# NoahVl/Explaining-In-Style-Reproducibility-Study

Hardware: AMD Instinct MI355X
Metric: StylEx G+D+enc train-step images/sec @256px (higher is better)
Workload: dtype bf16; 1 GPU; FFHQ-shaped 256x256 StylEx, batch 32/GPU, GAE=2 (noise+encoder micro-steps), GP every 4th step, ResNet-18 classifier; image_size=256, batch_per_gpu=32, start_step=0, gradient_accumulate_every=2, global_batch=32, parallelism=dp1

## Files before the change

### explaining-in-style-reproducibility-study_amd/csrc/conv_pipe.hip

```cpp
#include <hip/hip_runtime.h>
#include <stdint.h>
#include <stdlib.h>

#include "conv_prims.h"
#include "stylex_internal.h"

#ifndef PIPE_STORE_AUX
#define PIPE_STORE_AUX 0
#endif

struct StylexPipeArgs {
    int total_tiles;
    unsigned m_ntiles, m_tpi, m_tx;
    int dbg;
};

#ifdef STYLEX_PIPE_ABLATION
#define PIPE_DBG (pa.dbg)
#else
#define PIPE_DBG 0
#endif


namespace {

typedef StylexPipeArgs PipeArgs;

template <int NT>
struct PipeCfg {
    static constexpr int TH = NT == 128 ? 16 : 32;
    static constexpr int TW = 32, HWD = TW + 2, NP = (TH + 2) * HWD;
    static constexpr int H_PIECES = (NP + 31) / 32;
    static constexpr int H_STRIDE = H_PIECES * 1024;
    static constexpr int W_PIECES = 9 * NT / 32;
    static constexpr int W_STRIDE = W_PIECES * 1024;
    static constexpr int HS = 3, WS = 2;
    static constexpr int W_BASE = HS * H_STRIDE;
    static constexpr int BIAS_BASE = W_BASE + WS * W_STRIDE;
    static constexpr int DUMP_BASE = BIAS_BASE + 2048;
    static constexpr int SMEM = DUMP_BASE + 1024;
    static constexpr int HP_MAX = (H_PIECES + 7) / 8;
    static constexpr int WP_MAX = (W_PIECES + 7) / 8;
    static constexpr int RG = TH / 4;
};

__device__ __forceinline__ void lds_wait(bf16x8 (&av)[4], bf16x8 (&bv)[2]) {
    asm volatile("s_waitcnt lgkmcnt(0)" : "+v"(av[0]), "+v"(av[1]), "+v"(av[2]), "+v"(av[3]), "+v"(bv[0]), "+v"(bv[1]));
}
template <int HWD, int TAP>
__device__ __forceinline__ void tap_addr(int (&addr)[4], int a_base, unsigned& swz) {
    constexpr int kh = TAP / 3, kw = TAP % 3;
    asm volatile("" : "+v"(swz));
#pragma unroll
    for (int i = 0; i < 4; ++i) addr[i] = a_base + ((i + kh) * HWD + kw) * 32 + (int)(((swz >> ((i + kh) * 3 + kw)) & 1u) << 4);
}
template <int NT, int TAP>
__device__ __forceinline__ void load_tap(bf16x8 (&av)[4], bf16x8 (&bv)[2], const int (&addr)[4], int b_addr) {
    lds_read16<(TAP * NT) * 32>(bv[0], b_addr);
    lds_read16<(TAP * NT + 32) * 32>(bv[1], b_addr);
#pragma unroll
    for (int i = 0; i < 4; ++i) lds_read16<0>(av[i], addr[i]);
}

__device__ __forceinline__ void mfma8(f32x16 (&acc)[4][2], const bf16x8 (&av)[4], const bf16x8 (&bv)[2]) {
#pragma unroll
    for (int i = 0; i < 4; ++i)
#pragma unroll
        for (int j = 0; j < 2; ++j) mfma1(acc[i][j], bv[j], av[i]);
}

template <int NT, int EPI>
__global__ __launch_bounds__(512, 2) void conv3x3_pipe_kernel(ConvKParams p, PipeArgs pa) {
    using Cfg = PipeCfg<NT>;
    constexpr int TH = Cfg::TH, HWD = Cfg::HWD, NP = Cfg::NP, H_PIECES = Cfg::H_PIECES, H_STRIDE = Cfg::H_STRIDE;
    constexpr int W_PIECES = Cfg::W_PIECES, W_STRIDE = Cfg::W_STRIDE, W_BASE = Cfg::W_BASE;
    constexpr int HP_MAX = Cfg::HP_MAX, WP_MAX = Cfg::WP_MAX, RG = Cfg::RG;
    static_assert(WP_MAX + HP_MAX <= 9, "one DMA piece per tap");
    extern __shared__ __attribute__((aligned(16))) char smem[];
    const int tid = threadIdx.x, lane = tid & 63;
    const int wave = __builtin_amdgcn_readfirstlane(tid >> 6);
    const int H = p.Ho, W = p.Wo, C = p.Ck, N = p.N;
    const int n_tiles = N / NT;
    const int tiles_x = (W + 31) >> 5, tiles_y = (H + TH - 1) / TH;
    const int tpi = tiles_x * tiles_y;

    int xs, xn, bslot, nslots;
    xcd_tile_span(pa.total_tiles, xs, xn, bslot, nslots);
    if (bslot >= xn) return;
    for (int i = (bslot & 3) * (PIPE_DBG >> 8); i > 0; --i) __builtin_amdgcn_s_sleep(16);
    const int my_tiles = xcd_my_tiles(xn, bslot, nslots);
    const int nchunks = C >> 4;
    const int total = my_tiles * nchunks;

    auto decode = [&](int k, int& b, int& y0, int& x0, int& n0) {
        const int t = xs + bslot + k * nslots;
        int pt = fastdiv(t, pa.m_ntiles);
        n0 = (t - pt * n_tiles) * NT;
        b = fastdiv(pt, pa.m_tpi);
        pt -= b * tpi;
        const int ty = fastdiv(pt, pa.m_tx);
        y0 = ty * TH;
        x0 = (pt - ty * tiles_x) * 32;
    };

    const unsigned bytes_x = (unsigned)((long)p.B * H * W * C * 2);
    const unsigned bytes_w = (unsigned)((long)N * 9 * C * 2);
    const __amdgpu_buffer_rsrc_t rx = __builtin_amdgcn_make_buffer_rsrc(const_cast<float*>(p.a), 0, (int)bytes_x, 0x00020000);
    const __amdgpu_buffer_rsrc_t rw = __builtin_amdgcn_make_buffer_rsrc(const_cast<void*>(p.w), 0, (int)bytes_w, 0x00020000);
    constexpr unsigned OOB = 0x80000000u;

    const int lr = lane >> 1, pslot = lane & 1;
    const int half = pslot ^ ((lr >> 3) & 1);
    int h_dst[HP_MAX], w_dst[WP_MAX];
#pragma unroll
    for (int it = 0; it < HP_MAX; ++it) h_dst[it] = wave + 8 * it < H_PIECES ? (wave + 8 * it) * 1024 : -1;
    unsigned voff_h[HP_MAX];
    auto halo_voff = [&](int b, int y0, int x0) {
#pragma unroll
        for (int it = 0; it < HP_MAX; ++it) {
            const int piece = wave + 8 * it;
            const int hp = piece * 32 + lr;
            const int hh = hp / HWD, ww = hp - hh * HWD;
            const int y = y0 - 1 + hh, x = x0 - 1 + ww;
            const bool ok = piece < H_PIECES && hp < NP && y >= 0 && y < H && x >= 0 && x < W;
            voff_h[it] = ok ? ((unsigned)((b * H + y) * W + x) * (unsigned)C + (unsigned)half * 8u) * 2u : OOB;
        }
    };
    unsigned voff_w[WP_MAX];
#pragma unroll
    for (int it = 0; it < WP_MAX; ++it) {
        const int piece = wave + 8 * it;
        const int r = piece * 32 + lr;
        const int tap = r / NT, n = r - tap * NT;
        const int gt = p.flip_taps ? 8 - tap : tap;
        voff_w[it] = piece < W_PIECES ? ((unsigned)(n * 9 + gt) * (unsigned)C + (unsigned)half * 8u) * 2u : OOB;
        w_dst[it] = piece < W_PIECES ? piece * 1024 : -1;
    }
#define issue_h1(IT, STAGE, SOFF, MORE)                                                                              \
    dma16(rx, smem, h_dst[IT] >= 0 ? (STAGE) * H_STRIDE + h_dst[IT] : Cfg::DUMP_BASE, (MORE) ? voff_h[IT] : OOB, SOFF)
#define issue_w1(IT, WBUF, SOFF, MORE)                                                                               \
    dma16(rw, smem, w_dst[IT] >= 0 ? W_BASE + (WBUF) * W_STRIDE + w_dst[IT] : Cfg::DUMP_BASE, (MORE) ? voff_w[IT] : OOB, SOFF)

    const int rg = wave % RG, nh = wave / RG;
    const int li = lane & 31, lk = lane >> 5;
    const int a_row = (4 * rg) * HWD + li;
    int a_base = a_row * 32;
    unsigned swz = 0;
#pragma unroll
    for (int r = 0; r < 6; ++r)
#pragma unroll
        for (int kw = 0; kw < 3; ++kw) {
            const int t = a_row + r * HWD + kw;
            swz |= (unsigned)(((t >> 3) ^ lk) & 1) << (r * 3 + kw);
        }
    const int b_cur0 = W_BASE + (nh * 64 + li) * 32 + ((((li >> 3) ^ lk) & 1) << 4), b_cur1 = b_cur0 + W_STRIDE;

    if (EPI == 0 && (p.flags & STYLEX_EPI_BIAS) && tid < N) reinterpret_cast<float*>(smem + Cfg::BIAS_BASE)[tid] = p.bias[tid];

    f32x16 acc[4][2];
    auto zero_acc = [&]() {
#pragma unroll
        for (int i = 0; i < 4; ++i)
#pragma unroll
            for (int j = 0; j < 2; ++j)
#pragma unroll
                for (int e = 0; e < 16; ++e) acc[i][j][e] = 0.f;
    };
    zero_acc();

    const bool act = EPI == 0 && (p.flags & (STYLEX_EPI_LRELU | STYLEX_EPI_RELU)) != 0;
    const float slope = (p.flags & STYLEX_EPI_RELU) ? 0.f : 0.2f;
    const float gslope = p.res_scale;
    const bool mask_out = EPI == 0 && p.mask != nullptr;
    auto gatem = [&](unsigned u, unsigned bits) -> unsigned {
        const float a0 = __uint_as_float(u << 16), c0 = __uint_as_float(u & 0xffff0000u);
        f32x2_t t = {(bits & 1u) ? a0 : gslope * a0, (bits & 2u) ? c0 : gslope * c0};
        bf16x2_t r = __builtin_convertvector(t, bf16x2_t);
        return *reinterpret_cast<unsigned*>(&r);
    };
    auto gate2 = [&](unsigned u, unsigned g) -> unsigned {
        const float a0 = __uint_as_float(u << 16), c0 = __uint_as_float(u & 0xffff0000u);
        const float ga = __uint_as_float(g << 16), gc = __uint_as_float(g & 0xffff0000u);
        f32x2_t t = {ga > 0.f ? a0 : gslope * a0, gc > 0.f ? c0 : gslope * c0};
        bf16x2_t r = __builtin_convertvector(t, bf16x2_t);
        return *reinterpret_cast<unsigned*>(&r);
    };
    const unsigned bytes_y = (unsigned)((long)p.B * H * W * N * 2);
    const __amdgpu_buffer_rsrc_t ry = __builtin_amdgcn_make_buffer_rsrc(p.y, 0, (int)bytes_y, 0x00020000);
    const __amdgpu_buffer_rsrc_t rgate = __builtin_amdgcn_make_buffer_rsrc(const_cast<float*>(p.residual), 0, (int)bytes_y, 0x00020000);
    const __amdgpu_buffer_rsrc_t rmask = __builtin_amdgcn_make_buffer_rsrc(
        EPI == 2 ? const_cast<unsigned char*>(p.gate_mask) : p.mask, 0, (int)(bytes_y >> 4), 0x00020000);
    const unsigned rowb = (unsigned)(W * N) * 2u;
    auto pack2 = [](float a, float c) -> unsigned {
        f32x2_t t = {a, c};
        bf16x2_t r = __builtin_convertvector(t, bf16x2_t);
        return *reinterpret_cast<unsigned*>(&r);
    };
    const unsigned lane_off = (unsigned)(((4 * rg) * W + (lane & 7)) * N + nh * 64) * 2u +
                              (unsigned)(4 * ((lane >> 4) & 1) + 2 * ((lane >> 3) & 1) + (lane >> 5)) * 16u;
    const unsigned pixb8 = (unsigned)N * 16u;
    auto epilogue = [&](int b, int y0, int x0, int n0) {
        const int lh = lk;
        const int nb = n0 + nh * 64;
        const unsigned t_off = __builtin_amdgcn_readfirstlane((unsigned)((((long)(b * H + y0) * W + x0) * N + n0) * 2));
        const unsigned g_off = x0 + li < W ? (unsigned)(((4 * rg) * W + li) * N + nh * 64 + 8 * lh) * 2u : OOB;
#pragma unroll
        for (int i = 0; i < 4; ++i) {
            const bool row_ok = y0 + 4 * rg + i < H;
            const unsigned soff = t_off + i * rowb;
            u32x4 R[4];
#pragma unroll
            for (int j = 0; j < 2; ++j) {
                u32x4 gv[2];
                unsigned gm[2];
                if (EPI != 0) {
                    const unsigned voff = row_ok ? g_off : OOB;
#pragma unroll
                    for (int q = 0; q < 2; ++q) {
                        if (EPI == 1) gv[q] = __builtin_amdgcn_raw_buffer_load_b128(rgate, voff + (j * 64 + q * 32), soff, 0);
                        if (EPI == 2) gm[q] = __builtin_amdgcn_raw_buffer_load_b8(rmask, (voff >> 4) + (j * 4 + q * 2), soff >> 4, 0);
                    }
                }
                float4 b4[4];
#pragma unroll
                for (int g = 0; g < 4; ++g)
                    b4[g] = (EPI == 0 && (p.flags & STYLEX_EPI_BIAS))
                                ? *reinterpret_cast<const float4*>(smem + Cfg::BIAS_BASE + (nb + j * 32 + 8 * g + 4 * lh) * 4)
                                : make_float4(0.f, 0.f, 0.f, 0.f);
                unsigned P[4][2];
#pragma unroll
                for (int g = 0; g < 4; ++g) {
                    float v0 = acc[i][j][4 * g + 0] + b4[g].x, v1 = acc[i][j][4 * g + 1] + b4[g].y;
                    float v2 = acc[i][j][4 * g + 2] + b4[g].z, v3 = acc[i][j][4 * g + 3] + b4[g].w;
                    if (act) {
                        v0 = v0 > 0.f ? v0 : slope * v0;
                        v1 = v1 > 0.f ? v1 : slope * v1;
                        v2 = v2 > 0.f ? v2 : slope * v2;
                        v3 = v3 > 0.f ? v3 : slope * v3;
                    }
                    P[g][0] = pack2(v0, v1);
                    P[g][1] = pack2(v2, v3);
                }
#pragma unroll
                for (int g = 0; g < 4; g += 2)
#pragma unroll
                    for (int h = 0; h < 2; ++h) {
                        auto r = __builtin_amdgcn_permlane32_swap(P[g][h], P[g + 1][h], false, false);
                        P[g][h] = r[0];
                        P[g + 1][h] = r[1];
                    }
#pragma unroll
                for (int q = 0; q < 2; ++q) {
                    uint4 v = make_uint4(P[2 * q][0], P[2 * q][1], P[2 * q + 1][0], P[2 * q + 1][1]);
                    if (EPI == 1) {
                        v.x = gate2(v.x, gv[q].x);
                        v.y = gate2(v.y, gv[q].y);
                        v.z = gate2(v.z, gv[q].z);
                        v.w = gate2(v.w, gv[q].w);
                    } else if (EPI == 2) {
                        const unsigned m = gm[q];
                        v.x = gatem(v.x, m);
                        v.y = gatem(v.y, m >> 2);
                        v.z = gatem(v.z, m >> 4);
                        v.w = gatem(v.w, m >> 6);
                    }
                    if (mask_out && !(PIPE_DBG & 1))
                        __builtin_amdgcn_raw_buffer_store_b8((unsigned char)stylex_sign_bits8(v), rmask,
                                                             ((row_ok ? g_off : OOB) >> 4) + (j * 4 + q * 2), soff >> 4, 0);
                    R[2 * j + q] = u32x4{v.x, v.y, v.z, v.w};
                }
            }
#pragma unroll
            for (int j = 0; j < 2; ++j)
#pragma unroll
                for (int d = 0; d < 4; ++d) {
                    const unsigned a0 = R[2 * j][d], a1 = R[2 * j + 1][d];
                    R[2 * j][d] = (unsigned)__builtin_amdgcn_update_dpp((int)a0, (int)a1, 0x128, 0xF, 0xC, false);
                    R[2 * j + 1][d] = (unsigned)__builtin_amdgcn_update_dpp((int)a1, (int)a0, 0x128, 0xF, 0x3, false);
                }
#pragma unroll
            for (int q = 0; q < 2; ++q)
#pragma unroll
                for (int d = 0; d < 4; ++d) {
                    auto r = __builtin_amdgcn_permlane16_swap(R[q][d], R[2 + q][d], false, false);
                    R[q][d] = r[0];
                    R[2 + q][d] = r[1];
                }
            if (!(PIPE_DBG & 1)) {
#pragma unroll
                for (int k = 0; k < 4; ++k) {
                    const unsigned voff = (row_ok && x0 + 8 * k + (lane & 7) < W) ? lane_off : OOB;
                    __builtin_amdgcn_raw_buffer_store_b128(R[k], ry, voff, soff + k * pixb8, PIPE_STORE_AUX);
                    asm volatile("s_nop 1" : "+v"(R[k]) : : "memory");
                }
            }
        }
    };

    int hb, hy0, hx0, hn0;
    int h_k = 0, h_ch = 0, h_stage = 0;
    int w_k = 0, w_ch = 0, w_buf = 0, w_n0;
    int cb, cy0, cx0, cn0;
    decode(0, cb, cy0, cx0, cn0);
    hb = cb, hy0 = cy0, hx0 = cx0, hn0 = cn0;
    w_n0 = cn0;
    halo_voff(hb, hy0, hx0);
    auto adv_h = [&]() {
        h_stage = h_stage == 2 ? 0 : h_stage + 1;
        if (++h_ch == nchunks) {
            h_ch = 0;
            if (++h_k < my_tiles) {
                decode(h_k, hb, hy0, hx0, hn0);
                if (PIPE_DBG & 2) hb = 0, hy0 = 0, hx0 = 0;
                halo_voff(hb, hy0, hx0);
            }
        }
    };
    auto adv_w = [&]() {
        w_buf ^= 1;
        if (++w_ch == nchunks) {
            w_ch = 0;
            if (++w_k < my_tiles) {
                int b_, y_, x_;
                decode(w_k, b_, y_, x_, w_n0);
                if (PIPE_DBG & 4) w_n0 = 0;
            }
        }
    };
#pragma unroll
    for (int it = 0; it < HP_MAX; ++it) issue_h1(it, 0, 0u, true);
    adv_h();
#pragma unroll
    for (int it = 0; it < WP_MAX; ++it) issue_w1(it, 0, (unsigned)(w_n0 * 9 * C) * 2u, true);
    adv_w();
#pragma unroll
    for (int it = 0; it < HP_MAX; ++it) issue_h1(it, 1, (unsigned)h_ch * 32u, total > 1);
    if (total > 1) adv_h();

    int c_ch = 0, c_k = 0, c_stage = 0;
    bf16x8 avA[4], bvA[2], avB[4], bvB[2];
    int addr[4];
    tap_addr<HWD, 0>(addr, a_base, swz);
    wait_vmcnt<HP_MAX>();
    __builtin_amdgcn_s_barrier();
    asm volatile("" ::: "memory");
    load_tap<NT, 0>(avA, bvA, addr, b_cur0);
    tap_addr<HWD, 1>(addr, a_base, swz);
    auto next_stage = [&]() {
        a_base += c_stage == 2 ? -2 * H_STRIDE : H_STRIDE;
        c_stage = c_stage == 2 ? 0 : c_stage + 1;
    };
    constexpr int PPT = 2;
#define PIPE_DMA(TAP, MORE_W, MORE_H)                                                              \
    _Pragma("unroll") for (int q_ = (TAP) * PPT; q_ < (TAP) * PPT + PPT; ++q_) {                   \
        if (q_ < WP_MAX) issue_w1(q_, w_buf, w_soff, MORE_W);                                      \
        else if (q_ - WP_MAX < HP_MAX) issue_h1(q_ - WP_MAX, h_stage, h_soff, MORE_H);             \
    }
#define PIPE_TAP(TAP, AVC, BVC, AVN, BVN, BCUR, MORE_W, MORE_H) \
    lds_wait(AVC, BVC);                                        \
    load_tap<NT, TAP + 1>(AVN, BVN, addr, BCUR);               \
    __builtin_amdgcn_sched_barrier(0);                         \
    mfma8(acc, AVC, BVC);                                      \
    if (TAP == 7) next_stage();                                \
    tap_addr<HWD, (TAP + 2) % 9>(addr, a_base, swz);           \
    PIPE_DMA(TAP, MORE_W, MORE_H)                              \
    __builtin_amdgcn_sched_barrier(0);
#define PIPE_LAST(AVC, BVC, AVN, BVN, BNEXT)                   \
    lds_wait(AVC, BVC);                                        \
    if (PIPE_DBG & 8) wait_vmcnt<HP_MAX + 16>();                 \
    else wait_vmcnt<HP_MAX>();                                 \
    __builtin_amdgcn_s_barrier();                              \
    asm volatile("" ::: "memory");                             \
    load_tap<NT, 0>(AVN, BVN, addr, BNEXT);                    \
    __builtin_amdgcn_sched_barrier(0);                         \
    mfma8(acc, AVC, BVC);                                      \
    tap_addr<HWD, 1>(addr, a_base, swz);                       \
    __builtin_amdgcn_sched_barrier(0);
#define PIPE_CHUNK(A1, B1, A2, B2, BCUR, BNEXT, MORE_W, MORE_H)                                    \
    {                                                                                              \
        const bool mw_ = MORE_W, mh_ = MORE_H;                                                     \
        const unsigned w_soff = (unsigned)(w_n0 * 9 * C + w_ch * 16) * 2u, h_soff = (unsigned)h_ch * 32u; \
        PIPE_TAP(0, A1, B1, A2, B2, BCUR, mw_, mh_)                                                \
        PIPE_TAP(1, A2, B2, A1, B1, BCUR, mw_, mh_)                                                \
        PIPE_TAP(2, A1, B1, A2, B2, BCUR, mw_, mh_)                                                \
        PIPE_TAP(3, A2, B2, A1, B1, BCUR, mw_, mh_)                                                \
        PIPE_TAP(4, A1, B1, A2, B2, BCUR, mw_, mh_)                                                \
        PIPE_TAP(5, A2, B2, A1, B1, BCUR, mw_, mh_)                                                \
        PIPE_TAP(6, A1, B1, A2, B2, BCUR, mw_, mh_)                                                \
        PIPE_TAP(7, A2, B2, A1, B1, BCUR, mw_, mh_)                                                \
        PIPE_LAST(A1, B1, A2, B2, BNEXT)                                                           \
        if (mw_) adv_w();                                                                          \
        if (mh_) adv_h();                                                                          \
    }
    for (int g = 0; g < total; g += 2) {
        PIPE_CHUNK(avA, bvA, avB, bvB, b_cur0, b_cur1, g + 1 < total, g + 2 < total)
        PIPE_CHUNK(avB, bvB, avA, bvA, b_cur1, b_cur0, g + 2 < total, g + 3 < total)
        c_ch += 2;
        if (c_ch == nchunks) {
            c_ch = 0;
            asm volatile("s_nop 15\n\ts_nop 15"
                         : "+v"(acc[0][0]), "+v"(acc[0][1]), "+v"(acc[1][0]), "+v"(acc[1][1]), "+v"(acc[2][0]), "+v"(acc[2][1]),
                           "+v"(acc[3][0]), "+v"(acc[3][1]));
            epilogue(cb, cy0, cx0, cn0);
            if (++c_k < my_tiles) {
                decode(c_k, cb, cy0, cx0, cn0);
                zero_acc();
            }
        }
    }
#undef PIPE_CHUNK
#undef PIPE_LAST
#undef PIPE_TAP
#undef PIPE_DMA
#undef issue_h1
#undef issue_w1
    asm volatile("s_waitcnt lgkmcnt(0)" ::: "memory");
    wait_vmcnt<0>();
}

template <int NT, int EPI>
int launch_pipe(const ConvKParams& p, hipStream_t s) {
    using Cfg = PipeCfg<NT>;
    const hipError_t e = stylex_dynamic_lds_once<conv3x3_pipe_kernel<NT, EPI>>(Cfg::SMEM);
    if (e != hipSuccess) return (int)e;
    const int tiles_x = (p.Wo + 31) / 32, tiles_y = (p.Ho + Cfg::TH - 1) / Cfg::TH, n_tiles = p.N / NT;
    PipeArgs pa;
    pa.total_tiles = p.B * tiles_x * tiles_y * n_tiles;
    pa.m_ntiles = magic_of(n_tiles);
    pa.m_tpi = magic_of(tiles_x * tiles_y);
    pa.m_tx = magic_of(tiles_x);
#ifdef STYLEX_PIPE_ABLATION
    pa.dbg = getenv("STYLEX_PIPE_DBG") ? atoi(getenv("STYLEX_PIPE_DBG")) : 0;
#else
    pa.dbg = 0;
#endif
    stylex_note_kernel("conv3x3_pipe_kernel<%d, %d>", NT, EPI);
    hipLaunchKernelGGL((conv3x3_pipe_kernel<NT, EPI>), dim3((unsigned)stylex_cu_count()), dim3(512), Cfg::SMEM, s, p, pa);
    return (int)hipGetLastError();
}

template <int NT>
int launch_pipe_epi(const ConvKParams& p, hipStream_t s) {
    if (p.flags & STYLEX_EPI_GATE) return launch_pipe<NT, 1>(p, s);
    if (p.flags & STYLEX_EPI_GATE_MASK) return launch_pipe<NT, 2>(p, s);
    return launch_pipe<NT, 0>(p, s);
}

}

int stylex_launch_pipe(const ConvKParams& p, hipStream_t s) {
    const char* env = getenv("STYLEX_CONV_PIPE");
    if (env && env[0] == '0') return STYLEX_NOT_APPLICABLE;
    if (!p.act_bf16 || p.a_scale || p.s2d_c) return STYLEX_NOT_APPLICABLE;
    if (p.flags & ~(STYLEX_EPI_BIAS | STYLEX_EPI_LRELU | STYLEX_EPI_RELU | STYLEX_EPI_GATE | STYLEX_EPI_GATE_MASK | STYLEX_EPI_MASK_OUT))
        return STYLEX_NOT_APPLICABLE;
    if ((p.flags & STYLEX_EPI_GATE) && (!p.residual || (reinterpret_cast<uintptr_t>(p.residual) & 15))) return STYLEX_NOT_APPLICABLE;
    if (p.Ck < 64 || p.Ck % 32 != 0 || p.N % 64 != 0 || p.N > 512 || p.Wo < 32 || p.Ho < 16) return STYLEX_NOT_APPLICABLE;
    if ((reinterpret_cast<uintptr_t>(p.a) & 15) || (reinterpret_cast<uintptr_t>(p.w) & 15) || (reinterpret_cast<uintptr_t>(p.y) & 15))
        return STYLEX_NOT_APPLICABLE;
    if ((long)p.B * p.Ho * p.Wo * p.Ck * 2 >= (1l << 31) || (long)p.N * 9 * p.Ck * 2 >= (1l << 31) ||
        (long)p.B * p.Ho * p.Wo * p.N * 2 >= (1l << 31))
        return STYLEX_NOT_APPLICABLE;
    const bool n128 = p.N % 128 == 0 && !(env && env[0] == '6');
    if (!n128) {
        if (p.Ho < 32 && !(env && env[0] == '6')) return STYLEX_NOT_APPLICABLE;
        if (!(env && env[0] == '6') && ((p.flags & STYLEX_EPI_GATE) || (p.flip_taps && !p.flags && p.Ck == 64)))
            return STYLEX_NOT_APPLICABLE;
    }
    if (p.dry) return 0;
    if (n128) return launch_pipe_epi<128>(p, s);
    return launch_pipe_epi<64>(p, s);
}
```

### explaining-in-style-reproducibility-study_amd/csrc/conv_prims.h

```cpp
#pragma once
#include <hip/hip_runtime.h>

#include "act_io.h"

typedef float f32x16 __attribute__((ext_vector_type(16)));
typedef short bf16x8 __attribute__((ext_vector_type(8)));
typedef __bf16 bf16x2_t __attribute__((ext_vector_type(2)));
typedef float f32x2_t __attribute__((ext_vector_type(2)));
typedef unsigned u32x4 __attribute__((ext_vector_type(4)));
typedef __attribute__((address_space(3))) void* lds_void_ptr;

__device__ __forceinline__ void dma16(__amdgpu_buffer_rsrc_t r, char* smem, int lds_off, unsigned voff, unsigned soff = 0) {
    __builtin_amdgcn_raw_ptr_buffer_load_lds(r, (lds_void_ptr)(smem + lds_off), 16, voff, soff, 0, 0);
}

template <int N>
__device__ __forceinline__ void wait_vmcnt() {
    asm volatile("s_waitcnt vmcnt(%0)" ::"n"(N) : "memory");
}

template <int OFF>
__device__ __forceinline__ void lds_read16(bf16x8& dst, int addr) {
    asm volatile("ds_read_b128 %0, %1 offset:%2" : "=v"(dst) : "v"(addr), "n"(OFF));
}

__device__ __forceinline__ void mfma1(f32x16& acc, const bf16x8& a, const bf16x8& b) {
    asm volatile("v_mfma_f32_32x32x16_bf16 %0, %1, %2, %0" : "+v"(acc) : "v"(a), "v"(b));
}

__device__ __forceinline__ int fastdiv(int n, unsigned magic) { return magic ? (int)__umulhi((unsigned)n, magic) : n; }
inline unsigned magic_of(int d) { return d <= 1 ? 0u : (unsigned)(((1ull << 32) + (unsigned)d - 1) / (unsigned)d); }

__device__ __forceinline__ void xcd_tile_span(int total_tiles, int& xs, int& xn, int& bslot, int& nslots) {
    const int xcd = blockIdx.x & 7;
    bslot = blockIdx.x >> 3, nslots = gridDim.x >> 3;
    const int tq = total_tiles >> 3, tr = total_tiles & 7;
    xs = xcd * tq + (xcd < tr ? xcd : tr), xn = tq + (xcd < tr ? 1 : 0);
}
__device__ __forceinline__ int xcd_my_tiles(int xn, int bslot, int nslots) { return (xn - bslot + nslots - 1) / nslots; }
```

Measured before the change: 1003 images/sec.

## Add 16x16x32 MFMA variant of pipelined conv3x3 kernel for NT=128

New measurement: 1011 images/sec, median of 6. No clear change (+0.8%).

```diff
diff --git a/explaining-in-style-reproducibility-study_amd/csrc/conv_pipe.hip b/explaining-in-style-reproducibility-study_amd/csrc/conv_pipe.hip
--- a/explaining-in-style-reproducibility-study_amd/csrc/conv_pipe.hip
+++ b/explaining-in-style-reproducibility-study_amd/csrc/conv_pipe.hip
@@ -7,6 +7,10 @@
 
 #ifndef PIPE_STORE_AUX
 #define PIPE_STORE_AUX 0
+#endif
+
+#ifndef PIPE_MFMA
+#define PIPE_MFMA 0
 #endif
 
 struct StylexPipeArgs {
@@ -42,6 +46,7 @@
     static constexpr int HP_MAX = (H_PIECES + 7) / 8;
     static constexpr int WP_MAX = (W_PIECES + 7) / 8;
     static constexpr int RG = TH / 4;
+    static constexpr int mfma_n(int epi) { return PIPE_MFMA ? PIPE_MFMA : NT == 128 ? 16 : 32; }
 };
 
 __device__ __forceinline__ void lds_wait(bf16x8 (&av)[4], bf16x8 (&bv)[2]) {
@@ -70,7 +75,7 @@
 }
 
 template <int NT, int EPI>
-__global__ __launch_bounds__(512, 2) void conv3x3_pipe_kernel(ConvKParams p, PipeArgs pa) {
+__device__ __forceinline__ void pipe_body32(const ConvKParams& p, const PipeArgs& pa) {
     using Cfg = PipeCfg<NT>;
     constexpr int TH = Cfg::TH, HWD = Cfg::HWD, NP = Cfg::NP, H_PIECES = Cfg::H_PIECES, H_STRIDE = Cfg::H_STRIDE;
     constexpr int W_PIECES = Cfg::W_PIECES, W_STRIDE = Cfg::W_STRIDE, W_BASE = Cfg::W_BASE;
@@ -418,6 +423,424 @@
     wait_vmcnt<0>();
 }
 
+template <int HWD, int T>
+__device__ __forceinline__ void kstep_addr(int (&addr)[4], int a_base, int mid_delta, unsigned& swz, int& ls) {
+    constexpr int tA = (2 * T) % 9, tB = (2 * T + 1) % 9;
+    constexpr int offA = ((tA / 3) * HWD + tA % 3) * 32, offB = ((tB / 3) * HWD + tB % 3) * 32;
+    asm volatile("" : "+v"(swz), "+v"(ls));
+    const unsigned m = swz >> (tA + ls * (tB - tA));
+    int base = a_base + offA + ls * (offB - offA);
+    if (T == 4) base += ls * mid_delta;
+#pragma unroll
+    for (int i = 0; i < 4; ++i) addr[i] = base + i * HWD * 32 + (int)(((m >> (3 * i)) & 1u) << 4);
+}
+template <int OFF, int J0>
+__device__ __forceinline__ void load_w2(bf16x8 (&w)[4], int base) {
+    lds_read16<OFF + J0 * 512>(w[J0], base);
+    lds_read16<OFF + J0 * 512 + 512>(w[J0 + 1], base);
+}
+template <int I0>
+__device__ __forceinline__ void load_x4(bf16x8 (&x)[4], const int (&addr)[4]) {
+    lds_read16<0>(x[0], addr[I0]);
+    lds_read16<512>(x[1], addr[I0]);
+    lds_read16<0>(x[2], addr[I0 + 1]);
+    lds_read16<512>(x[3], addr[I0 + 1]);
+}
+__device__ __forceinline__ void lds_wait0(bf16x8 (&w)[4], bf16x8 (&x)[4]) {
+    asm volatile("s_waitcnt lgkmcnt(0)" : "+v"(w[0]), "+v"(w[1]), "+v"(w[2]), "+v"(w[3]), "+v"(x[0]), "+v"(x[1]), "+v"(x[2]), "+v"(x[3]));
+}
+__device__ __forceinline__ void lds_wait1(bf16x8 (&x)[4], bf16x8 (&wn)[4]) {
+    asm volatile("s_waitcnt lgkmcnt(0)" : "+v"(x[0]), "+v"(x[1]), "+v"(x[2]), "+v"(x[3]), "+v"(wn[0]), "+v"(wn[1]));
+}
+template <int P0>
+__device__ __forceinline__ void mfma16x16(f32x4 (&acc)[8][4], const bf16x8 (&w)[4], const bf16x8 (&x)[4]) {
+#pragma unroll
+    for (int q = 0; q < 4; ++q)
+#pragma unroll
+        for (int j = 0; j < 4; ++j) mfma16(acc[P0 + q][j], w[j], x[q]);
+}
+
+template <int NT, int EPI>
+__device__ __forceinline__ void pipe_body16(const ConvKParams& p, const PipeArgs& pa) {
+    using Cfg = PipeCfg<NT>;
+    constexpr int TH = Cfg::TH, HWD = Cfg::HWD, NP = Cfg::NP, H_PIECES = Cfg::H_PIECES, H_STRIDE = Cfg::H_STRIDE;
+    constexpr int W_PIECES = Cfg::W_PIECES, W_STRIDE = Cfg::W_STRIDE, W_BASE = Cfg::W_BASE;
+    constexpr int HP_MAX = Cfg::HP_MAX, WP_MAX = Cfg::WP_MAX, RG = Cfg::RG;
+    static_assert(WP_MAX + HP_MAX <= 9, "a phase's DMA pieces fit three half-steps");
+    extern __shared__ __attribute__((aligned(16))) char smem[];
+    const int tid = threadIdx.x, lane = tid & 63;
+    const int wave = __builtin_amdgcn_readfirstlane(tid >> 6);
+    const int H = p.Ho, W = p.Wo, C = p.Ck, N = p.N;
+    const int n_tiles = N / NT;
+    const int tiles_x = (W + 31) >> 5, tiles_y = (H + TH - 1) / TH;
+    const int tpi = tiles_x * tiles_y;
+
+    int xs, xn, bslot, nslots;
+    xcd_tile_span(pa.total_tiles, xs, xn, bslot, nslots);
+    if (bslot >= xn) return;
+    for (int i = (bslot & 3) * (PIPE_DBG >> 8); i > 0; --i) __builtin_amdgcn_s_sleep(16);
+    const int my_tiles = xcd_my_tiles(xn, bslot, nslots);
+    const int nchunks = C >> 4;
+    const int total = my_tiles * nchunks;
+
+    auto decode = [&](int k, int& b, int& y0, int& x0, int& n0) {
+        const int t = xs + bslot + k * nslots;
+        int pt = fastdiv(t, pa.m_ntiles);
+        n0 = (t - pt * n_tiles) * NT;
+        b = fastdiv(pt, pa.m_tpi);
+        pt -= b * tpi;
+        const int ty = fastdiv(pt, pa.m_tx);
+        y0 = ty * TH;
+        x0 = (pt - ty * tiles_x) * 32;
+    };
+
+    const unsigned bytes_x = (unsigned)((long)p.B * H * W * C * 2);
+    const unsigned bytes_w = (unsigned)((long)N * 9 * C * 2);
+    const __amdgpu_buffer_rsrc_t rx = __builtin_amdgcn_make_buffer_rsrc(const_cast<float*>(p.a), 0, (int)bytes_x, 0x00020000);
+    const __amdgpu_buffer_rsrc_t rw = __builtin_amdgcn_make_buffer_rsrc(const_cast<void*>(p.w), 0, (int)bytes_w, 0x00020000);
+    constexpr unsigned OOB = 0x80000000u;
+
+    const int lr = lane >> 1, pslot = lane & 1;
+    const int half = pslot ^ ((lr >> 3) & 1);
+    int h_dst[HP_MAX], w_dst[WP_MAX];
+#pragma unroll
+    for (int it = 0; it < HP_MAX; ++it) h_dst[it] = wave + 8 * it < H_PIECES ? (wave + 8 * it) * 1024 : -1;
+    unsigned voff_h[HP_MAX];
+    auto halo_voff = [&](int b, int y0, int x0) {
+#pragma unroll
+        for (int it = 0; it < HP_MAX; ++it) {
+            const int piece = wave + 8 * it;
+            const int hp = piece * 32 + lr;
+            const int hh = hp / HWD, ww = hp - hh * HWD;
+            const int y = y0 - 1 + hh, x = x0 - 1 + ww;
+            const bool ok = piece < H_PIECES && hp < NP && y >= 0 && y < H && x >= 0 && x < W;
+            voff_h[it] = ok ? ((unsigned)((b * H + y) * W + x) * (unsigned)C + (unsigned)half * 8u) * 2u : OOB;
+        }
+    };
+    unsigned voff_w[WP_MAX];
+#pragma unroll
+    for (int it = 0; it < WP_MAX; ++it) {
+        const int piece = wave + 8 * it;
+        const int r = piece * 32 + lr;
+        const int tap = r / NT, n = r - tap * NT;
+        const int gt = p.flip_taps ? 8 - tap : tap;
+        voff_w[it] = piece < W_PIECES ? ((unsigned)(n * 9 + gt) * (unsigned)C + (unsigned)half * 8u) * 2u : OOB;
+        w_dst[it] = piece < W_PIECES ? piece * 1024 : -1;
+    }
+#define issue_h1(IT, STAGE, SOFF, MORE)                                                                              \
+    dma16(rx, smem, h_dst[IT] >= 0 ? (STAGE) * H_STRIDE + h_dst[IT] : Cfg::DUMP_BASE, (MORE) ? voff_h[IT] : OOB, SOFF)
+#define issue_w1(IT, WBUF, SOFF, MORE)                                                                               \
+    dma16(rw, smem, w_dst[IT] >= 0 ? W_BASE + (WBUF) * W_STRIDE + w_dst[IT] : Cfg::DUMP_BASE, (MORE) ? voff_w[IT] : OOB, SOFF)
+
+    const int rg = wave % RG, nh = wave / RG;
+    const int lc = lane & 15, lh = (lane >> 4) & 1;
+    int ls = lane >> 5;
+    const int pc = lc ^ (lc < 8 ? 4 : 0);
+    const int a_row = (4 * rg) * HWD + pc;
+    int a_base = a_row * 32;
+    unsigned swz = 0;
+#pragma unroll
+    for (int r = 0; r < 6; ++r)
+#pragma unroll
+        for (int kw = 0; kw < 3; ++kw) {
+            const int t = a_row + r * HWD + kw;
+            swz |= (unsigned)(((t >> 3) ^ lh) & 1) << (r * 3 + kw);
+        }
+    const int b_0 = W_BASE + (nh * 64 + pc) * 32 + ((((pc >> 3) ^ lh) & 1) << 4);
+    const int b_s0 = b_0 + ls * (NT * 32), b_s1 = b_s0 + W_STRIDE;
+    const int b_mid = ls ? b_0 + W_STRIDE : b_0 + 8 * NT * 32;
+
+    if (EPI == 0 && (p.flags & STYLEX_EPI_BIAS) && tid < N) reinterpret_cast<float*>(smem + Cfg::BIAS_BASE)[tid] = p.bias[tid];
+
+    f32x4 acc[8][4];
+    auto zero_acc = [&]() {
+#pragma unroll
+        for (int q = 0; q < 8; ++q)
+#pragma unroll
+            for (int j = 0; j < 4; ++j)
+#pragma unroll
+                for (int e = 0; e < 4; ++e) acc[q][j][e] = 0.f;
+    };
+    zero_acc();
+
+    const bool act = EPI == 0 && (p.flags & (STYLEX_EPI_LRELU | STYLEX_EPI_RELU)) != 0;
+    const float slope = (p.flags & STYLEX_EPI_RELU) ? 0.f : 0.2f;
+    const float gslope = p.res_scale;
+    const bool mask_out = EPI == 0 && p.mask != nullptr;
+    auto gatem = [&](unsigned u, unsigned bits) -> unsigned {
+        const float a0 = __uint_as_float(u << 16), c0 = __uint_as_float(u & 0xffff0000u);
+        f32x2_t t = {(bits & 1u) ? a0 : gslope * a0, (bits & 2u) ? c0 : gslope * c0};
+        bf16x2_t r = __builtin_convertvector(t, bf16x2_t);
+        return *reinterpret_cast<unsigned*>(&r);
+    };
+    auto gate2 = [&](unsigned u, unsigned g) -> unsigned {
+        const float a0 = __uint_as_float(u << 16), c0 = __uint_as_float(u & 0xffff0000u);
+        const float ga = __uint_as_float(g << 16), gc = __uint_as_float(g & 0xffff0000u);
+        f32x2_t t = {ga > 0.f ? a0 : gslope * a0, gc > 0.f ? c0 : gslope * c0};
+        bf16x2_t r = __builtin_convertvector(t, bf16x2_t);
+        return *reinterpret_cast<unsigned*>(&r);
+    };
+    const unsigned bytes_y = (unsigned)((long)p.B * H * W * N * 2);
+    const __amdgpu_buffer_rsrc_t ry = __builtin_amdgcn_make_buffer_rsrc(p.y, 0, (int)bytes_y, 0x00020000);
+    const __amdgpu_buffer_rsrc_t rgate = __builtin_amdgcn_make_buffer_rsrc(const_cast<float*>(p.residual), 0, (int)bytes_y, 0x00020000);
+    const __amdgpu_buffer_rsrc_t rmask = __builtin_amdgcn_make_buffer_rsrc(
+        EPI == 2 ? const_cast<unsigned char*>(p.gate_mask) : p.mask, 0, (int)(bytes_y >> 4), 0x00020000);
+    const unsigned rowb = (unsigned)(W * N) * 2u;
+    auto pack2 = [](float a, float c) -> unsigned {
+        f32x2_t t = {a, c};
+        bf16x2_t r = __builtin_convertvector(t, bf16x2_t);
+        return *reinterpret_cast<unsigned*>(&r);
+    };
+    const bool lo32 = lane < 32;
+    const int quad = (lane >> 4) ^ (lane < 32 ? 1 : 0);
+    const unsigned g_base = (unsigned)(((4 * rg) * W + pc) * N + nh * 64) * 2u + (unsigned)(4 * lh + ls) * 16u;
+    const unsigned l_ch = (unsigned)(nh * 64) * 2u + (unsigned)(2 * ((lane >> 3) & 1) + 4 * lh + ls) * 16u;
+    const int px_t[2] = {(lane & 7) ^ 4, lane & 7};
+    const unsigned lane_off[2] = {(unsigned)(((4 * rg) * W + px_t[0]) * N) * 2u + l_ch, (unsigned)(((4 * rg) * W + px_t[1]) * N) * 2u + l_ch};
+    const unsigned pixb8 = (unsigned)N * 16u;
+    auto epilogue = [&](int b, int y0, int x0, int n0) {
+        const int nb = n0 + nh * 64;
+        const unsigned t_off = __builtin_amdgcn_readfirstlane((unsigned)((((long)(b * H + y0) * W + x0) * N + n0) * 2));
+        unsigned gm[2][2][2];
+        auto load_gm = [&](int i) {
+#pragma unroll
+            for (int pp = 0; pp < 2; ++pp)
+#pragma unroll
+                for (int m = 0; m < 2; ++m) {
+                    const unsigned g_off = (y0 + 4 * rg + i < H && x0 + 16 * pp + pc < W) ? g_base : OOB;
+                    gm[i & 1][pp][m] = __builtin_amdgcn_raw_buffer_load_b8(rmask, (g_off >> 4) + m * 2, (t_off + i * rowb + pp * 2 * pixb8) >> 4, 0);
+                }
+        };
+        if (EPI == 2) load_gm(0);
+#pragma unroll
+        for (int i = 0; i < 4; ++i) {
+            const bool row_ok = y0 + 4 * rg + i < H;
+            if (EPI == 2 && i < 3) load_gm(i + 1);
+            float4 b4[4];
+#pragma unroll
+            for (int j = 0; j < 4; ++j)
+                b4[j] = (EPI == 0 && (p.flags & STYLEX_EPI_BIAS))
+                            ? *reinterpret_cast<const float4*>(smem + Cfg::BIAS_BASE + (nb + 16 * j + 4 * quad) * 4)
+                            : make_float4(0.f, 0.f, 0.f, 0.f);
+#pragma unroll
+            for (int pp = 0; pp < 2; ++pp) {
+                const int q = 2 * i + pp;
+                const unsigned soff = t_off + i * rowb + pp * 2 * pixb8;
+                const unsigned g_off = (row_ok && x0 + 16 * pp + pc < W) ? g_base : OOB;
+                u32x4 gv[2];
+                if (EPI == 1) {
+#pragma unroll
+                    for (int m = 0; m < 2; ++m) gv[m] = __builtin_amdgcn_raw_buffer_load_b128(rgate, g_off + m * 32, soff, 0);
+                }
+                u32x4 R[2];
+#pragma unroll
+                for (int m = 0; m < 2; ++m) {
+                    unsigned P[2][2];
+#pragma unroll
+                    for (int jl = 0; jl < 2; ++jl) {
+                        const int j = m + 2 * jl;
+                        float v0 = acc[q][j][0] + b4[j].x, v1 = acc[q][j][1] + b4[j].y;
+                        float v2 = acc[q][j][2] + b4[j].z, v3 = acc[q][j][3] + b4[j].w;
+                        if (act) {
+                            v0 = v0 > 0.f ? v0 : slope * v0;
+                            v1 = v1 > 0.f ? v1 : slope * v1;
+                            v2 = v2 > 0.f ? v2 : slope * v2;
+                            v3 = v3 > 0.f ? v3 : slope * v3;
+                        }
+                        P[jl][0] = pack2(v0, v1);
+                        P[jl][1] = pack2(v2, v3);
+                    }
+#pragma unroll
+                    for (int d = 0; d < 2; ++d) {
+                        auto r = __builtin_amdgcn_permlane16_swap(P[0][d], P[1][d], false, false);
+                        P[0][d] = r[0];
+                        P[1][d] = r[1];
+                    }
+                    uint4 v = make_uint4(lo32 ? P[1][0] : P[0][0], lo32 ? P[1][1] : P[0][1], lo32 ? P[0][0] : P[1][0], lo32 ? P[0][1] : P[1][1]);
+                    if (EPI == 1) {
+                        v.x = gate2(v.x, gv[m].x);
+                        v.y = gate2(v.y, gv[m].y);
+                        v.z = gate2(v.z, gv[m].z);
+                        v.w = gate2(v.w, gv[m].w);
+                    } else if (EPI == 2) {
+                        const unsigned mb = gm[i & 1][pp][m];
+                        v.x = gatem(v.x, mb);
+                        v.y = gatem(v.y, mb >> 2);
+                        v.z = gatem(v.z, mb >> 4);
+                        v.w = gatem(v.w, mb >> 6);
+                    }
+                    if (mask_out && !(PIPE_DBG & 1))
+                        __builtin_amdgcn_raw_buffer_store_b8((unsigned char)stylex_sign_bits8(v), rmask, (g_off >> 4) + m * 2, soff >> 4, 0);
+                    R[m] = u32x4{v.x, v.y, v.z, v.w};
+                }
+#pragma unroll
+                for (int d = 0; d < 4; ++d) {
+                    const unsigned a0 = R[0][d], a1 = R[1][d];
+                    R[0][d] = (unsigned)__builtin_amdgcn_update_dpp((int)a0, (int)a1, 0x128, 0xF, 0xC, false);
+                    R[1][d] = (unsigned)__builtin_amdgcn_update_dpp((int)a1, (int)a0, 0x128, 0xF, 0x3, false);
+                }
+                if (!(PIPE_DBG & 1)) {
+#pragma unroll
+                    for (int k = 0; k < 2; ++k) {
+                        const unsigned voff = (row_ok && x0 + 16 * pp + 8 * k + px_t[k] < W) ? lane_off[k] : OOB;
+                        __builtin_amdgcn_raw_buffer_store_b128(R[k], ry, voff, soff + k * pixb8, PIPE_STORE_AUX);
+                        asm volatile("s_nop 1" : "+v"(R[k]) : : "memory");
+                    }
+                }
+            }
+        }
+    };
+
+    int hb, hy0, hx0, hn0;
+    int h_k = 0, h_ch = 0, h_stage = 0;
+    int w_k = 0, w_ch = 0, w_buf = 0, w_n0;
+    int cb, cy0, cx0, cn0;
+    decode(0, cb, cy0, cx0, cn0);
+    hb = cb, hy0 = cy0, hx0 = cx0, hn0 = cn0;
+    w_n0 = cn0;
+    halo_voff(hb, hy0, hx0);
+    auto adv_h = [&]() {
+        h_stage = h_stage == 2 ? 0 : h_stage + 1;
+        if (++h_ch == nchunks) {
+            h_ch = 0;
+            if (++h_k < my_tiles) {
+                decode(h_k, hb, hy0, hx0, hn0);
+                if (PIPE_DBG & 2) hb = 0, hy0 = 0, hx0 = 0;
+                halo_voff(hb, hy0, hx0);
+            }
+        }
+    };
+    auto adv_w = [&]() {
+        w_buf ^= 1;
+        if (++w_ch == nchunks) {
+            w_ch = 0;
+            if (++w_k < my_tiles) {
+                int b_, y_, x_;
+                decode(w_k, b_, y_, x_, w_n0);
+                if (PIPE_DBG & 4) w_n0 = 0;
+            }
+        }
+    };
+#pragma unroll
+    for (int it = 0; it < HP_MAX; ++it) issue_h1(it, 0, 0u, true);
+    adv_h();
+#pragma unroll
+    for (int it = 0; it < WP_MAX; ++it) issue_w1(it, 0, (unsigned)(w_n0 * 9 * C) * 2u, true);
+    adv_w();
+#pragma unroll
+    for (int it = 0; it < HP_MAX; ++it) issue_h1(it, 1, (unsigned)h_ch * 32u, total > 1);
+    if (total > 1) adv_h();
+
+    int c_ch = 0, c_k = 0, c_stage = 0;
+    bf16x8 wA[4], wB[4], xl[4], xh[4];
+    int addr[4];
+    auto stage_delta = [&]() { return c_stage == 2 ? -2 * H_STRIDE : H_STRIDE; };
+    auto next_stage = [&]() {
+        a_base += stage_delta();
+        c_stage = c_stage == 2 ? 0 : c_stage + 1;
+    };
+    kstep_addr<HWD, 0>(addr, a_base, 0, swz, ls);
+    wait_vmcnt<HP_MAX>();
+    __builtin_amdgcn_s_barrier();
+    asm volatile("" ::: "memory");
+    load_w2<0, 0>(wA, b_s0);
+    load_w2<0, 2>(wA, b_s0);
+    load_x4<0>(xl, addr);
+#define W_BASE_OF(T) ((T) < 4 ? b_s0 : (T) == 4 ? b_mid : b_s1)
+#define W_IMM_OF(T) ((T) < 4 ? 2 * (T) * NT * 32 : (T) == 4 ? 0 : (2 * (T) - 9) * NT * 32)
+#define PIPE_DMA(SLOT, MORE_W, MORE_H)                                                             \
+    _Pragma("unroll") for (int q_ = (SLOT) * 3; q_ < (SLOT) * 3 + 3; ++q_) {                       \
+        if (q_ < WP_MAX) issue_w1(q_, w_buf, w_soff, MORE_W);                                      \
+        else if (q_ - WP_MAX < HP_MAX) issue_h1(q_ - WP_MAX, h_stage, h_soff, MORE_H);             \
+    }
+#define PIPE_SOFFS w_soff = (unsigned)(w_n0 * 9 * C + w_ch * 16) * 2u, h_soff = (unsigned)h_ch * 32u;
+#define PIPE_ADV(MORE_W, MORE_H) \
+    if (MORE_W) adv_w();         \
+    if (MORE_H) adv_h();
+#define PIPE_KSTEP(T, TN, WC, WN)                                                                  \
+    lds_wait0(WC, xl);                                                                             \
+    load_x4<2>(xh, addr);                                                                          \
+    if (T != 3 && T != 8) load_w2<W_IMM_OF(TN), 0>(WN, W_BASE_OF(TN));                              \
+    __builtin_amdgcn_sched_barrier(0);                                                             \
+    mfma16x16<0>(acc, WC, xl);                                                                     \
+    if (T == 4 || T == 8) next_stage();                                                            \
+    kstep_addr<HWD, TN>(addr, a_base, stage_delta(), swz, ls);                                     \
+    if (T == 0) { PIPE_SOFFS PIPE_DMA(0, mwA, mhA) }                                               \
+    if (T == 1) { PIPE_DMA(2, mwA, mhA) PIPE_ADV(mwA, mhA) }                                       \
+    if (T == 5) { PIPE_DMA(1, mwB, mhB) }                                                          \
+    __builtin_amdgcn_sched_barrier(0);                                                             \
+    lds_wait1(xh, WN);                                                                             \
+    if (T == 3 || T == 8) {                                                                        \
+        if (PIPE_DBG & 8) wait_vmcnt<HP_MAX + 16>();                                               \
+        else wait_vmcnt<HP_MAX>();                                                                 \
+    }                                                                                              \
+    if (T == 3 || T == 4 || T == 8) {                                                              \
+        __builtin_amdgcn_s_barrier();                                                              \
+        asm volatile("" ::: "memory");                                                             \
+    }                                                                                              \
+    load_x4<0>(xl, addr);                                                                          \
+    if (T == 3 || T == 8) load_w2<W_IMM_OF(TN), 0>(WN, W_BASE_OF(TN));                              \
+    load_w2<W_IMM_OF(TN), 2>(WN, W_BASE_OF(TN));                                                    \
+    __builtin_amdgcn_sched_barrier(0);                                                             \
+    mfma16x16<4>(acc, WC, xh);                                                                     \
+    if (T == 0) { PIPE_DMA(1, mwA, mhA) }                                                          \
+    if (T == 4) { PIPE_SOFFS PIPE_DMA(0, mwB, mhB) }                                               \
+    if (T == 5) { PIPE_DMA(2, mwB, mhB) PIPE_ADV(mwB, mhB) }                                       \
+    __builtin_amdgcn_sched_barrier(0);
+#define PIPE_ITER(W0, W1)          \
+    PIPE_KSTEP(0, 1, W0, W1)       \
+    PIPE_KSTEP(1, 2, W1, W0)       \
+    PIPE_KSTEP(2, 3, W0, W1)       \
+    PIPE_KSTEP(3, 4, W1, W0)       \
+    PIPE_KSTEP(4, 5, W0, W1)       \
+    PIPE_KSTEP(5, 6, W1, W0)       \
+    PIPE_KSTEP(6, 7, W0, W1)       \
+    PIPE_KSTEP(7, 8, W1, W0)       \
+    PIPE_KSTEP(8, 0, W0, W1)
+    for (int g = 0; g < total; g += 2) {
+        const bool mwA = g + 1 < total, mhA = g + 2 < total, mwB = g + 2 < total, mhB = g + 3 < total;
+        unsigned w_soff, h_soff;
+        PIPE_ITER(wA, wB)
+        lds_wait0(wB, xl);
+#pragma unroll
+        for (int j = 0; j < 4; ++j) wA[j] = wB[j];
+        c_ch += 2;
+        if (c_ch == nchunks) {
+            c_ch = 0;
+            asm volatile("s_nop 15\n\ts_nop 15"
+                         : "+v"(acc[0][0]), "+v"(acc[0][1]), "+v"(acc[0][2]), "+v"(acc[0][3]), "+v"(acc[1][0]), "+v"(acc[1][1]),
+                           "+v"(acc[1][2]), "+v"(acc[1][3]), "+v"(acc[2][0]), "+v"(acc[2][1]), "+v"(acc[2][2]), "+v"(acc[2][3]),
+                           "+v"(acc[3][0]), "+v"(acc[3][1]), "+v"(acc[3][2]), "+v"(acc[3][3]));
+            asm volatile(""
+                         : "+v"(acc[4][0]), "+v"(acc[4][1]), "+v"(acc[4][2]), "+v"(acc[4][3]), "+v"(acc[5][0]), "+v"(acc[5][1]),
+                           "+v"(acc[5][2]), "+v"(acc[5][3]), "+v"(acc[6][0]), "+v"(acc[6][1]), "+v"(acc[6][2]), "+v"(acc[6][3]),
+                           "+v"(acc[7][0]), "+v"(acc[7][1]), "+v"(acc[7][2]), "+v"(acc[7][3]));
+            epilogue(cb, cy0, cx0, cn0);
+            if (++c_k < my_tiles) {
+                decode(c_k, cb, cy0, cx0, cn0);
+                zero_acc();
+            }
+        }
+    }
+#undef PIPE_ITER
+#undef PIPE_KSTEP
+#undef PIPE_ADV
+#undef PIPE_SOFFS
+#undef PIPE_DMA
+#undef W_IMM_OF
+#undef W_BASE_OF
+#undef issue_h1
+#undef issue_w1
+    asm volatile("s_waitcnt lgkmcnt(0)" ::: "memory");
+    wait_vmcnt<0>();
+}
+
+template <int NT, int EPI>
+__global__ __launch_bounds__(512, 2) void conv3x3_pipe_kernel(ConvKParams p, PipeArgs pa) {
+    if constexpr (PipeCfg<NT>::mfma_n(EPI) == 16) pipe_body16<NT, EPI>(p, pa);
+    else pipe_body32<NT, EPI>(p, pa);
+}
+
 template <int NT, int EPI>
 int launch_pipe(const ConvKParams& p, hipStream_t s) {
     using Cfg = PipeCfg<NT>;
diff --git a/explaining-in-style-reproducibility-study_amd/csrc/conv_prims.h b/explaining-in-style-reproducibility-study_amd/csrc/conv_prims.h
--- a/explaining-in-style-reproducibility-study_amd/csrc/conv_prims.h
+++ b/explaining-in-style-reproducibility-study_amd/csrc/conv_prims.h
@@ -4,6 +4,7 @@
 #include "act_io.h"
 
 typedef float f32x16 __attribute__((ext_vector_type(16)));
+typedef float f32x4 __attribute__((ext_vector_type(4)));
 typedef short bf16x8 __attribute__((ext_vector_type(8)));
 typedef __bf16 bf16x2_t __attribute__((ext_vector_type(2)));
 typedef float f32x2_t __attribute__((ext_vector_type(2)));
@@ -28,6 +29,10 @@
     asm volatile("v_mfma_f32_32x32x16_bf16 %0, %1, %2, %0" : "+v"(acc) : "v"(a), "v"(b));
 }
 
+__device__ __forceinline__ void mfma16(f32x4& acc, const bf16x8& a, const bf16x8& b) {
+    asm volatile("v_mfma_f32_16x16x32_bf16 %0, %1, %2, %0" : "+v"(acc) : "v"(a), "v"(b));
+}
+
 __device__ __forceinline__ int fastdiv(int n, unsigned magic) { return magic ? (int)__umulhi((unsigned)n, magic) : n; }
 inline unsigned magic_of(int d) { return d <= 1 ? 0u : (unsigned)(((1ull << 32) + (unsigned)d - 1) / (unsigned)d); }
 
```
